# Keyteer/Mixed-precision_LU_Factorization

Measured on AMD Instinct MI355X. Metric: LU GFLOP/s at N=32768 (1/2/4/8 GPUs); IR iterations to ||r||/||b||<1e-12, higher is better.
Workload: dtype f64

## Files before the change

### mixed-precision_lu_factorization_amd/csrc/mpf_host.cpp

```cpp
#include "mpf_internal.h"
#include "../../include/MPF.h"
#include <climits>
#include <cstdio>
#include <cstdlib>
#include <cstring>
#include <cmath>
#include <iostream>
#include <vector>
#include <mutex>
#include <functional>
#include <chrono>

static thread_local std::string g_noctx_err;

namespace {
struct OptDesc { const char *name, *env; size_t off; bool wide; long long lo, hi; };
#define OPT_I(field, env, lo, hi) {#field, env, offsetof(MpfTuning, field), false, lo, hi}
#define OPT_L(field, env, lo, hi) {#field, env, offsetof(MpfTuning, field), true, lo, hi}
const OptDesc kOpts[] = {
    OPT_I(safe_pivots, "MPF_SAFE_PIVOTS", 0, 1),
    OPT_I(chain_pipeline, "MPF_CHAIN_PIPELINE", 0, 1),
    OPT_L(chain_pipeline_below, "MPF_CHAIN_PIPELINE_BELOW", 0, 1ll << 40),
    OPT_I(fp16_work32, "MPF_FP16_WORK32", 0, 1),
    OPT_I(superpanel_fp16, "MPF_SUPERPANEL", 0, 8),
    OPT_I(superpanel_fp64, "MPF_SUPERPANEL_FP64", 1, 8),
    OPT_I(no_lookahead, "MPF_NO_LOOKAHEAD", 0, 1),
    OPT_I(verbose, "MPF_VERBOSE", 0, 1),
    OPT_I(timeline, "MPF_TIMELINE", 0, 1),
    OPT_L(hp_spin_limit, "MPF_HP_SPIN_LIMIT", 1, 1ll << 31),
    OPT_L(hp_gate_ticks, "MPF_HP_GATE_TICKS", 0, 1ll << 40),
    OPT_I(hp_acq_fence, "MPF_HP_ACQ_FENCE", 0, 1),
    OPT_I(hp_window, "MPF_HP_WINDOW", -1, 1 << 30),
    OPT_I(hgemm_pad, "MPF_HGEMM_PAD", 0, 65536),
    OPT_I(hgemm_split_pad, "MPF_HGEMM_SPLIT_PAD", 0, 65536),
    OPT_I(hgemm_big, "MPF_HGEMM_BIG", 0, 1),
    OPT_I(hgemm_big_tile, "MPF_HGEMM_BIG_TILE", 0, 5),
    OPT_I(hgemm_mfma16, "MPF_HGEMM_MFMA16", 0, 1),
    OPT_I(dgemm_dma, "MPF_DGEMM_DMA", 0, 1),
    OPT_I(lazy_gather, "MPF_LAZY_GATHER", 0, 1),
    OPT_I(dpanel_fused_form, "MPF_DPANEL_FUSED", 0, 1),
    OPT_I(dist_instalments, "MPF_DIST_INSTALMENTS", 0, 1),
    OPT_L(dist_instalment_min_bytes, "MPF_DIST_INSTALMENT_MIN_BYTES", 0, 1ll << 40),
    OPT_I(generic_fused, "MPF_GENERIC_FUSED", 0, 1),
    OPT_I(fp64_rowmajor, "MPF_FP64_ROWMAJOR", 0, 1),
    OPT_L(fp64_rowmajor_min_n, "MPF_FP64_ROWMAJOR_MIN_N", 0, 1ll << 40),
    OPT_I(trsm_laswp_fused, "MPF_TRSM_LASWP_FUSED", 0, 1),
    OPT_I(fp64_two_lanes, "MPF_FP64_TWO_LANES", 0, 1 << 30),
    OPT_I(fp64_lane_a_pct, "MPF_FP64_LANE_A_PCT", 20, 90),
    OPT_I(event_timers, "MPF_EVENT_TIMERS", 0, 2),
    OPT_I(dist_world1_loop, "MPF_DIST_WORLD1_LOOP", 0, 1),
    OPT_I(gesv_fp64_tflops, "MPF_GESV_FP64_TFLOPS", 0, 1000),
    OPT_I(gate_wait_value, "MPF_GATE_WAIT_VALUE", 0, 1),
    OPT_I(host_sink, "MPF_HOST_SINK", 0, 1),
    OPT_I(sink_trace, "MPF_SINK_TRACE", 0, 1),
    OPT_I(hp_half_slabs, "MPF_HP_HALF_SLABS", 0, 1),
    OPT_I(hp_half_slabs_rows, "MPF_HP_HALF_SLABS_ROWS", 256, 32768),
    OPT_I(hp_local_xcd, "MPF_HP_LOCAL_XCD", 0, 2),
    OPT_I(host_late_parts, "MPF_HOST_LATE_PARTS", 0, 4),
    OPT_L(host_late_min_n, "MPF_HOST_LATE_MIN_N", 0, 1ll << 40),
    OPT_I(host_first_pct, "MPF_HOST_FIRST_PCT", 5, 100),
    OPT_I(host_late_q_pct, "MPF_HOST_LATE_Q_PCT", 1, 1000),
    OPT_L(host_sink_min_n, "MPF_HOST_SINK_MIN_N", 0, 1ll << 40),
    OPT_I(dist_solve_p2p, "MPF_DIST_SOLVE_P2P", 0, 1),
#ifdef MPF_PROBE
    OPT_I(hp_stamp, "MPF_HP_STAMP", 0, 1),
    OPT_I(hp_r256_upto, "MPF_HP_R256_UPTO", 0, 1 << 30),
    OPT_I(dgemm_w8, "MPF_DGEMM_W8", 0, 1),
    OPT_I(gemm_lds_pad, "MPF_GEMM_LDS_PAD", 0, 65536),
    OPT_I(hgemm_big_reg, "MPF_HGEMM_BIG_REG", 0, 1),
    OPT_I(hgemm_dbg, "MPF_HGEMM_DBG", 0, 8191),
#endif
};
#undef OPT_I
#undef OPT_L
void opt_store(MpfTuning &t, const OptDesc &d, long long v) {
    if (v < d.lo) v = d.lo;
    if (v > d.hi) v = d.hi;
    char *p = (char *)&t + d.off;
    if (d.wide) *(long long *)p = v; else *(int *)p = (int)v;
}
long long opt_load(const MpfTuning &t, const OptDesc &d) {
    const char *p = (const char *)&t + d.off;
    return d.wide ? *(const long long *)p : (long long)*(const int *)p;
}
void tuning_from_env(MpfTuning &t) {
    for (const OptDesc &d : kOpts)
        if (const char *e = getenv(d.env)) if (*e) opt_store(t, d, atoll(e));
}
}

static int fail(mpf_ctx *c, int code, const std::string &msg) {
    if (c) c->err = msg; else g_noctx_err = msg;
    return code;
}

extern "C" {

int mpf_create(mpf_ctx **out, int device) {
    if (!out) return -1;
    *out = nullptr;
    int ndev = 0;
    hipError_t e = hipGetDeviceCount(&ndev);
    if (e != hipSuccess || ndev == 0) return fail(nullptr, -3, "No HIP devices available.");
    if (device < 0 || device >= ndev) return fail(nullptr, -1, "mpf_create: bad device index");
    mpf_ctx *c = new mpf_ctx();
    tuning_from_env(c->tune);
    c->device = device;
    if (hipSetDevice(device) != hipSuccess) { delete c; return fail(nullptr, -2, "hipSetDevice failed"); }
    hipDeviceProp_t prop;
    if (hipGetDeviceProperties(&prop, device) == hipSuccess) c->num_cus = prop.multiProcessorCount;
    if (hipStreamCreateWithFlags(&c->stream, hipStreamNonBlocking) != hipSuccess) { delete c; return fail(nullptr, -2, "hipStreamCreate failed"); }
    c->own_stream = true;
    {
        int lo = 0, hi = 0;
        hipDeviceGetStreamPriorityRange(&lo, &hi);
        if (hipStreamCreateWithPriority(&c->pstream, hipStreamNonBlocking, hi) != hipSuccess) c->pstream = nullptr;
        if (hipStreamCreateWithPriority(&c->tstream, hipStreamNonBlocking, hi) != hipSuccess) c->tstream = nullptr;
    }
    if (hipMalloc((void **)&c->ws, sizeof(MpfWorkspace)) != hipSuccess) { hipStreamDestroy(c->stream); delete c; return fail(nullptr, -2, "hipMalloc(workspace) failed"); }
    hipMemset(c->ws, 0, sizeof(MpfWorkspace));
    if (hipExtMallocWithFlags((void **)&c->hp_signal, 8, hipMallocSignalMemory) != hipSuccess) { c->hp_signal = nullptr; (void)hipGetLastError(); }
    else hipMemset(c->hp_signal, 0, 8);
    hipEventCreate(&c->ev0);
    hipEventCreate(&c->ev1);
    *out = c;
    return 0;
}

int mpf_destroy(mpf_ctx *c) {
    if (!c) return 0;
    hipSetDevice(c->device);
// ... 381 lines not shown
                if (!e) e = launch_laswp_from_list(c, d_A, lda, first, c->lists);
                if (!e) e = launch_dgetf2_npv(c, d_A, lda, pr, pc, o.fused_panel, 0);
                return e;
            });
            st.panels++;
        }
    }
    for (int64_t k = 0; k < N && rc == 0; k += nb) {
        const int pc = (int)((N - k) < nb ? (N - k) : nb);
        if (N - k <= 1 || k + pc >= N) break;
        const int64_t n = N - k - pc;
        const int64_t nx = k + pc;
        const int pc2 = (int)((N - nx) < nb ? (N - nx) : nb);
        const bool has_next = (N - nx) > 1;
        double *Ap = d_A + k * lda + k;
        double *A12 = d_A + nx * lda + k;
        const int64_t ns = has_next ? pc2 : n;
        rc = ev.timed(st.ms_trsm, S, [&] { return launch_dtrsm_llnu(c, pc, ns, Ap, lda, A12, lda); });
        if (rc) break;
        rc = ev.timed(st.ms_gemm, S, [&] {
            int e = o.trailing != MPF_TRAIL_FP64 ? launch_cvt_l21(c, Ap + pc, lda, n, pc, o.trailing == MPF_TRAIL_FP16X3) : 0;
            if (!e) e = trail_gemm(c, o, n, ns, pc, Ap + pc, A12, A12 + pc, lda);
            return e; });
        if (rc) break;
        count_gemm(st, o, n, ns, pc);
        if (!has_next) break;
        hipEvent_t e1 = ev.get(), e2 = ev.get();
        hipEventRecord(e1, S);
        hipEvent_t e2p = nullptr, e2t = nullptr;
        int rcp = 0;
        const bool piped = chain_pipelined(c, ev, st, o, d_A, lda, N, nx, pc2, d_ipiv, c->lists + (nx / nb), e1, &e2p, &e2t, &rcp) == 0;
        if (piped) rc = rcp;
        else {
            hipStreamWaitEvent(P, e1, 0);
            StreamSwap sw(c, P);
            double *Anx = d_A + nx * lda + nx;
            MovedList *ml = c->lists + (nx / nb);
            rc = ev.timed(st.ms_hpanel, P, [&] {
                return launch_hgetf2(c, Anx, lda, nullptr, 0, (int)(N - nx), pc2, (int)nx, d_ipiv + nx, nullptr, 0, ml, 0, o.trailing == MPF_TRAIL_FP64 ? HP_FP64_WINDOW_ROWS : 0); });
            if (!rc) rc = ev.timed(st.ms_dpanel, P, [&] {
                int e = launch_laswp_from_list(c, d_A + nx * lda, lda, pc2, ml);
                if (!e) e = launch_dgetf2_npv(c, Anx, lda, (int)(N - nx), pc2, o.fused_panel, (int)nx);
                return e;
            });
        }
        if (rc) break;
        if (!piped) hipEventRecord(e2, P);
        st.panels++;
        if (n > pc2) {
            rc = ev.timed(st.ms_laswp, S, [&] {
                return launch_laswp_from_list(c, d_A + (nx + pc2) * lda, lda, N - nx - pc2, c->lists + (k / nb)); });
            if (rc) break;
            double *A12r = A12 + (int64_t)pc2 * lda;
            rc = ev.timed(st.ms_trsm, S, [&] { return launch_dtrsm_llnu(c, pc, n - pc2, Ap, lda, A12r, lda); });
            if (rc) break;
            if (sink) sink_notify(c, (int)(k / nb) + 1, S);
            rc = ev.timed(st.ms_gemm, S, [&] { return trail_gemm(c, o, n, n - pc2, pc, Ap + pc, A12r, A12r + pc, lda); });
            if (rc) break;
            count_gemm(st, o, n, n - pc2, pc);
        }
        if (piped) { hipStreamWaitEvent(S, e2p, 0); hipStreamWaitEvent(S, e2t, 0); }
        else hipStreamWaitEvent(S, e2, 0);
        rc = ev.timed(st.ms_laswp, S, [&] {
            const int64_t s0 = nx + pc2;
            const int64_t sw = (N - s0) < nb ? (N - s0) : nb;
            return sw > 0 ? launch_laswp_from_list(c, d_A + s0 * lda, lda, sw, c->lists + (nx / nb)) : 0;
        });
        if (o.verbose) printf("panel k=%lld rows=%lld cols=%d (look-ahead)\n", (long long)nx, (long long)(N - nx), pc2);
    }
    if (sink) {
        hipEvent_t ep = ev.get(); hipEventRecord(ep, P); hipStreamWaitEvent(S, ep, 0);
        sink_notify(c, (int)((N + nb - 1) / nb), S);
    } else if (!rc) rc = ev.timed(st.ms_laswp, S, [&] { return launch_lazy_left_swaps(c, d_A, lda, N, nb, (int)((N + nb - 1) / nb), c->lists); });
    hipError_t se = sink_stream_wait(c, S);
    hipError_t sp = sink_stream_wait(c, P);
    if (c->tstream) { const hipError_t stt = sink_stream_wait(c, c->tstream); if (sp == hipSuccess) sp = stt; }
    if (!rc && (se != hipSuccess || sp != hipSuccess))
        return fail(c, -2, std::string("factorization failed: ") + hipGetErrorString(se != hipSuccess ? se : sp));
    ev.collect();
    st.lookahead = 1;
    return rc;
}

static int factor_lookahead_rm(mpf_ctx *c, double *d_A, int64_t lda, int64_t N, int32_t nb, int32_t *d_ipiv,
                               const mpf_opts &o, mpf_stats &st) {
    hipStream_t S = c->stream, P = c->pstream, T = c->tstream;
    EvPool ev(c);
    ev.keep = &st.ms_gemm;
    int rc = 0;
    const bool sink = sink_take(c, d_A, lda, N, nb);
    double *R = c->r64;
    const int64_t ldr = N;
    LatePlan *lp = (c->late && !c->late->taken && c->late->nseg > 0 && lda == N) ? c->late : nullptr;
    if (lp) lp->taken = true;
    int lseg = 0;
    int64_t ce = lp ? lp->c0[0] : N;
    { hipEvent_t e = ev.get(); hipEventRecord(e, S); hipStreamWaitEvent(P, e, 0); if (T) hipStreamWaitEvent(T, e, 0); }
    const int pc0 = (int)(N < nb ? N : nb);
    hipEvent_t chain_a = nullptr, chain_b = nullptr;
    if (N > 1) {
        hipEvent_t e0 = ev.get();
        {
            StreamSwap sw(c, P);
            rc = ev.timed(st.ms_hpanel, P, [&] {
                int e = launch_hgetf2(c, d_A, lda, nullptr, 0, (int)N, pc0, 0, d_ipiv, nullptr, 0, c->lists, 0, o.trailing == MPF_TRAIL_FP64 ? HP_FP64_WINDOW_ROWS : 0);
                if (!e) e = launch_laswp_from_list(c, d_A, lda, pc0, c->lists);
                if (!e) e = launch_dgetf2_npv(c, d_A, lda, (int)N, pc0, o.fused_panel, 0);
                return e; });
            hipEventRecord(e0, P);
        }
        st.panels++;
        if (!rc && pc0 < ce) rc = ev.timed(st.ms_cvt, S, [&] { return launch_transpose64(c, d_A + (int64_t)pc0 * lda, lda, R + pc0, ldr, N, ce - pc0, true); });
        hipStreamWaitEvent(S, e0, 0);
        chain_a = e0;
    }
    int64_t cm = -1;
    hipEvent_t doneL = nullptr, doneR = nullptr, prevR = nullptr;
    hipEvent_t init_done = ev.get();
    hipEventRecord(init_done, S);
    bool was_two = false;
    for (int64_t k = 0; k < N && rc == 0; k += nb) {
        const int pc = (int)((N - k) < nb ? (N - k) : nb);
        if (N - k <= 1 || k + pc >= N) break;
        const int64_t n = N - k - pc;
        const int64_t nx = k + pc;
        const int pc2 = (int)((N - nx) < nb ? (N - nx) : nb);
        const bool has_next = (N - nx) > 1;
        double *Ap = d_A + k * lda + k;
        double *LT = c->rm_lt + ((k / nb) & 1) * N * (int64_t)nb;
        const int64_t ns = has_next ? pc2 : n;
        MovedList *lk = c->lists + (k / nb);
        while (lp && lseg < lp->nseg && (k / nb >= lp->q[lseg] || nx + pc2 > ce || !has_next)) {
            const int64_t c_lo = lp->c0[lseg], c_hi = lseg + 1 < lp->nseg ? lp->c0[lseg + 1] : N, w = c_hi - c_lo;
            double *LT3 = c->rm_lt + 2 * N * (int64_t)nb;
            rc = launch_late_wait(c, lp->flags + lseg, lp->seq);
            if (!rc && lp->snapshot) {
                MPF_HIP_TRY(c, hipMemcpyAsync(lp->snapshot + c_lo * N, d_A + c_lo * lda, (size_t)w * N * sizeof(double), hipMemcpyDeviceToDevice, S));
                lp->snapped[lseg] = true;
            }
            if (!rc) rc = ev.timed(st.ms_cvt, S, [&] { return launch_transpose64(c, d_A + c_lo * lda, lda, R + c_lo, ldr, N, w, true); });
            for (int64_t kj = 0; kj < k && rc == 0; kj += nb) {
                const int64_t nxj = kj + nb, nj = N - nxj;
                double *Apj = d_A + kj * lda + kj;
                const MovedList *lj = c->lists + (kj / nb);
                rc = ev.timed(st.ms_cvt, S, [&] { return launch_transpose64(c, Apj + nb, lda, LT3, nb, nj, nb, true); });
                if (!rc) rc = ev.timed(st.ms_laswp, S, [&] { return launch_laswp_from_list_rm64(c, R + c_lo, ldr, w, lj, (int64_t)LASWP_MAXMOVED * c_lo); });
                if (!rc) rc = ev.timed(st.ms_trsm, S, [&] { return launch_dtrsm_llnu_strided(c, nb, w, Apj, lda, R + kj * ldr + c_lo, ldr, 1); });
                if (!rc) rc = ev.timed(st.ms_cvt, S, [&] { return launch_transpose64(c, d_A + c_lo * lda + kj, lda, R + kj * ldr + c_lo, ldr, nb, w, false); });
                if (!rc) rc = ev.timed(st.ms_gemm, S, [&] { return launch_dgemm_minus(c, w, nj, nb, R + kj * ldr + c_lo, ldr, LT3, nb, R + nxj * ldr + c_lo, ldr); });
                count_gemm(st, o, nj, w, nb);
                if (sink && !rc && c_hi == N) sink_notify(c, (int)(kj / nb) + 1, S);
            }
            ++lseg;
            ce = lseg < lp->nseg ? lp->c0[lseg] : N;
            cm = -1;
            doneR = ev.get();
            hipEventRecord(doneR, S);
            doneL = nullptr;
        }
        if (rc) break;
        const int64_t cw = ce - nx - pc2;
        const bool pivots_fit = c->num_cus <= 0 || (N - nx + HP_R - 1) / HP_R <= (int64_t)c->num_cus * 4 / 5;
        const bool want_two = T && c->tune.fp64_two_lanes > 0 && has_next && pivots_fit && (N - nx) > c->tune.chain_pipeline_below &&
                              cw >= c->tune.fp64_two_lanes;
        bool resplit = false;
        if (!want_two) cm = -1;
        else if (cm < 0 || (cm - (nx + pc2)) * 100 < cw * (c->tune.fp64_lane_a_pct - 10)) {
            cm = nx + pc2 + ((cw * c->tune.fp64_lane_a_pct / 100 + 127) / 128) * 128;
            if (cm > ce - 128) cm = ce - 128;
            resplit = true;
        }
        if (cm >= 0) {
            const int64_t aw = cm - (nx + pc2);
            if (!was_two && k > 0) {
                doneL = ev.get();
                hipEventRecord(doneL, S);
            }
            hipEvent_t lt_ready = ev.get();
            {
                if (prevR) hipStreamWaitEvent(P, prevR, 0);
                StreamSwap sw(c, P);
                rc = ev.timed(st.ms_cvt, P, [&] { return launch_transpose64(c, Ap + pc, lda, LT, pc, n, pc, true); });
                hipEventRecord(lt_ready, P);
            }
            if (rc) break;
            hipEvent_t e1 = ev.get(), e2 = ev.get(), evA = ev.get(), evB = ev.get();
            {
                if (chain_a) hipStreamWaitEvent(T, chain_a, 0);
                if (chain_b) hipStreamWaitEvent(T, chain_b, 0);
                if (doneL) hipStreamWaitEvent(T, doneL, 0); else hipStreamWaitEvent(T, init_done, 0);
                if (resplit && doneR) hipStreamWaitEvent(T, doneR, 0);
                StreamSwap sw(c, T);
                rc = ev.timed(st.ms_laswp, T, [&] { return launch_laswp_from_list_rm64(c, R + nx, ldr, cm - nx, lk); });
                if (!rc) rc = ev.timed(st.ms_trsm, T, [&] { return launch_dtrsm_llnu_strided(c, pc, ns, Ap, lda, R + k * ldr + nx, ldr, 1); });
                hipStreamWaitEvent(T, lt_ready, 0);
                if (!rc) rc = ev.timed(st.ms_gemm, T, [&] { return launch_dgemm_minus(c, ns, n, pc, R + k * ldr + nx, ldr, LT, pc, R + nx * ldr + nx, ldr); });
                count_gemm(st, o, n, ns, pc);
                if (!rc) rc = ev.timed(st.ms_cvt, T, [&] { return launch_transpose64(c, d_A + nx * lda + nx, lda, R + nx * ldr + nx, ldr, N - nx, pc2, false); });
                hipEventRecord(e1, T);
            }
            if (rc) break;
            {
                hipStreamWaitEvent(P, e1, 0);
                if (doneR) hipStreamWaitEvent(P, doneR, 0);
// ... 323 lines not shown
            if (!rc && overlap) { e1 = ev.get(); hipEventRecord(e1, Ci); }
            if (!rc) rc = inner_step(k, pc, nx + sw_, e1c - nx - sw_, false);
            if (!rc && N - nx > 1) rc = side_chain(nx, e1, e2);
            if (!rc) rc = far_tasks_upto(it + 1);
            if (rc) break;
            if (nx >= c1 && far.on) {
                const int64_t c2 = (c1 + sbw) < N ? (c1 + sbw) : N;
                const int64_t e2c = inner_end(c2);
                if (!rc && !f64) rc = ev.timed(st.ms_cvt, S, [&] { return launch_cvt_l21(c, d_A + c0 * lda + c1, lda, N - c1, (int)(c1 - c0), split, far.img); });
                if (!rc) rc = big_update(far, e1c, e2c - e1c);
                if (!rc) rc = back_to_f64(c1, e1c, e2c - e1c);
                if (lanes) { ni_ready = ev.get(); hipEventRecord(ni_ready, S); }
                if (!rc) rc = big_update(far, e2c, N - e2c);
                if (rc) break;
            }
            if (overlap) { if (e2) { if (lanes) chain_done = e2; else hipStreamWaitEvent(S, e2, 0); } }
            if (o.verbose) printf("panel k=%lld rows=%lld (super-panel [%lld, %lld))\n", (long long)nx, (long long)(N - nx), (long long)c0, (long long)c1);
        }
        if (stop) break;
    }
    if (lanes) { hipEvent_t e = ev.get(); hipEventRecord(e, Ci); hipStreamWaitEvent(S, e, 0); if (chain_done) hipStreamWaitEvent(S, chain_done, 0); }
    if (!rc) rc = ev.timed(st.ms_laswp, S, [&] { return launch_lazy_left_swaps(c, d_A, lda, N, nb, (int)((N + nb - 1) / nb), c->lists, sb); });
    hipError_t se = hipStreamSynchronize(S);
    hipError_t sp = overlap ? hipStreamSynchronize(P) : hipSuccess;
    if (overlap && c->tstream) { const hipError_t stt = hipStreamSynchronize(c->tstream); if (sp == hipSuccess) sp = stt; }
    if (lanes) { const hipError_t sc = hipStreamSynchronize(Ci); if (sp == hipSuccess) sp = sc; }
    if (!rc && (se != hipSuccess || sp != hipSuccess))
        return fail(c, -2, std::string("factorization failed: ") + hipGetErrorString(se != hipSuccess ? se : sp));
    ev.collect();
    st.lookahead = overlap ? 1 : 0;
    return rc;
}

int mpf_ensure_rowmajor_copy(mpf_ctx *c, int64_t N, int64_t cols, int32_t nb) {
    const bool bad = c->r64.grow(N * cols) || c->rm_tmp.grow((int64_t)LASWP_MAXMOVED * cols) ||
                     c->rm_lt.grow(3 * N * (int64_t)nb);
    if (bad) {
        (void)hipGetLastError();
        c->r64.release(); c->rm_tmp.release(); c->rm_lt.release();
        return 1;
    }
    return 0;
}

int mpf_factor_setup(mpf_ctx *c, int64_t N, int32_t nb, int32_t npanels, bool lists) {
    if (lists) {
        MPF_HIP_TRY(c, c->lists.grow(npanels));
        MPF_HIP_TRY(c, c->perm_tmp.grow(N * (int64_t)(nb > HP_MAXCOLS ? nb : HP_MAXCOLS)));
        MPF_HIP_TRY(c, c->Fmap.grow(2 * N));
        MPF_HIP_TRY(c, hipMemsetAsync(c->lists, 0, (size_t)npanels * sizeof(MovedList), c->stream));
    }
    const int imax = INT_MAX;
    MPF_HIP_TRY(c, hipMemcpyAsync(&c->ws->info, &imax, sizeof(int), hipMemcpyHostToDevice, c->stream));
    MPF_HIP_TRY(c, hipMemsetAsync(&c->ws->hp_timeouts, 0, sizeof(int), c->stream));
    return 0;
}

int mpf_factor_dev(mpf_ctx *c, double *d_A, int64_t lda, int64_t N, int32_t nb, int32_t *d_ipiv, const mpf_opts *opts) {
    if (!c || !d_A || !d_ipiv) return -1;
    if (N <= 0 || nb <= 0) return fail(c, -1, "mpf_factor: N and panel width must be positive");
    if (lda < N) return fail(c, -1, "mpf_factor: lda < N");
    if (N > INT_MAX / 2) return fail(c, -1, "mpf_factor: N too large");
    if (nb > 65535) return fail(c, -1, "mpf_factor: panel width > 65535");
    mpf_opts o{};
    if (opts) o = *opts;
    if (o.trailing < MPF_TRAIL_FP64 || o.trailing > MPF_TRAIL_FP16X3) return fail(c, -1, "mpf_factor: unknown trailing mode");
    MPF_HIP_TRY(c, hipSetDevice(c->device));
    const bool force_generic = o.pivot_path == 1 || safe_pivots(c);
    const bool generic = force_generic || !hgetf2_lds_eligible(c, (int)N, (int)(nb < N ? nb : N));
    int want_sb = o.trailing != MPF_TRAIL_FP64 ? c->tune.superpanel_fp16 : c->tune.superpanel_fp64;
    if (o.trailing != MPF_TRAIL_FP64 && want_sb == 0) want_sb = (o.trailing == MPF_TRAIL_FP16 && N >= 24576) ? 6 : 4;
    if (o.superpanel > 0) want_sb = o.superpanel > 8 ? 8 : o.superpanel;
    const int sb = (!generic && !o.sync_timing && (int64_t)want_sb * nb < N) ? want_sb : 1;
    if (o.trailing != MPF_TRAIL_FP64) {
        const int64_t kimg = (int64_t)sb * nb < 8 * HP_MAXCOLS ? (int64_t)sb * nb : 8 * HP_MAXCOLS;
        int e = mpf_ensure_h_images(c, N + HP_MAXCOLS + 64, (int)kimg, sb > 1); if (e) return e;
    }
    { const int e = mpf_factor_setup(c, N, nb, (int)((N + nb - 1) / nb), !generic); if (e) return e; }
    mpf_stats st{};
    st.n = N; st.nb = nb; st.superpanel = sb;
    const bool lookahead = !o.sync_timing && !o.no_lookahead && !c->tune.no_lookahead && c->pstream != nullptr;
    const bool use_rm = !generic && sb <= 1 && lookahead && o.trailing == MPF_TRAIL_FP64 && c->tune.fp64_rowmajor &&
                        N >= c->tune.fp64_rowmajor_min_n && N > nb && mpf_ensure_rowmajor_copy(c, N, N, nb) == 0;
    if (c->late && !use_rm) {
        const int e = feed_finish(c);
        c->late = nullptr;
        if (e) return e;
    }
    MPF_HIP_TRY(c, hipEventRecord(c->ev0, c->stream));
    int rc;
    if (generic) rc = factor_generic(c, d_A, lda, N, nb, d_ipiv, o, st, force_generic);
    else if (sb > 1) rc = factor_superpanel(c, d_A, lda, N, nb, d_ipiv, o, st, sb, lookahead);
    else if (use_rm) rc = factor_lookahead_rm(c, d_A, lda, N, nb, d_ipiv, o, st);
    else if (lookahead) rc = factor_lookahead(c, d_A, lda, N, nb, d_ipiv, o, st);
    else {
        mpf_opts o2 = o;
        rc = factor_sync_timed(c, d_A, lda, N, nb, d_ipiv, o2, st);
    }
    hipEventRecord(c->ev1, c->stream);
    hipError_t se = sink_stream_wait(c, c->stream);
    if (rc) return rc;
    if (se != hipSuccess) return fail(c, -2, std::string("factorization failed: ") + hipGetErrorString(se));
    float ms = 0;
    hipEventElapsedTime(&ms, c->ev0, c->ev1);
    st.ms_total = ms;
    if (o.trailing == MPF_TRAIL_FP64 && N >= 8192 && ms > 0)
        c->fp64_rate_tflops = 2.0 / 3.0 * (double)N * (double)N * (double)N / (ms * 1e-3) / 1e12;
    int info = 0, flags0 = 0;
    MPF_HIP_TRY(c, hipMemcpy(&info, &c->ws->info, sizeof(int), hipMemcpyDeviceToHost));
    MPF_HIP_TRY(c, hipMemcpy(&flags0, &c->ws->hp_timeouts, sizeof(int), hipMemcpyDeviceToHost));
    st.info = info == INT_MAX ? 0 : info;
    st.hpanel_timeouts = flags0;
    const double h2d = c->stats.ms_h2d, d2h = c->stats.ms_d2h;
    c->stats = st;
    c->stats.ms_h2d = h2d; c->stats.ms_d2h = d2h;
    if (flags0) return fail(c, -4, "fp16 pivot kernel: inter-workgroup hand-off timed out (its workgroups were not all resident: GPU "
                                   "shared with another process?).  d_A and ipiv are invalid.  Use mpf_opts.pivot_path = 1 or MPF_SAFE_PIVOTS=1");
    return st.info;
}

static int ensure_host_copies(mpf_ctx *c, int64_t N) {
    MPF_HIP_TRY(c, c->host_A.grow(N * N));
    MPF_HIP_TRY(c, c->host_P.grow(N));
    return 0;
}

int mpf_trim(mpf_ctx *c) {
    if (!c) return -1;
    MPF_HIP_TRY(c, hipSetDevice(c->device));
    MPF_HIP_TRY(c, hipStreamSynchronize(c->stream));
    c->host_A.release(); c->host_P.release(); c->host_A0.release();
    sink_trim(c);
    feed_trim(c);
    c->r64.release(); c->rm_tmp.release(); c->rm_lt.release();
    c->w32.release();
    return 0;
}

int mpf_factor_host(mpf_ctx *c, double *A_host, int64_t N, int32_t nb, int32_t *ipiv_host, const mpf_opts *opts) {
    if (!c || !A_host || !ipiv_host) return -1;
    if (N <= 0 || nb <= 0) return fail(c, -1, "mpf_factor: N and panel width must be positive");
    MPF_HIP_TRY(c, hipSetDevice(c->device));
    { const int e = ensure_host_copies(c, N); if (e) return e; }
    double *dA = c->host_A;
    int32_t *dP = c->host_P;
    const size_t bytes = (size_t)N * (size_t)N * sizeof(double), pbytes = (size_t)N * sizeof(int32_t);
    const bool want_sink = c->tune.host_sink && N >= c->tune.host_sink_min_n && c->pstream != nullptr && !(opts && (opts->sync_timing || opts->no_lookahead)) &&
                           !(opts && opts->trailing != MPF_TRAIL_FP64) && !(opts && opts->pivot_path == 1);
    bool armed = false;
    if (want_sink) {
        if (c->host_A0.grow((int64_t)((bytes + pbytes + sizeof(double) - 1) / sizeof(double))) != hipSuccess)
            (void)hipGetLastError();
        if (c->host_A0) {
            const int e = sink_attach(c, A_host, N, nb);
            if (e < 0) return e;
            armed = e == 0;
        }
    }
    LatePlan plan;
    const int64_t npan = (N + nb - 1) / nb;
    int parts = c->tune.host_late_parts;
    if (!want_sink || !c->tune.fp64_rowmajor || N < c->tune.fp64_rowmajor_min_n || N < c->tune.host_late_min_n || npan < 32 || c->tune.no_lookahead || safe_pivots(c) ||
        !hgetf2_lds_eligible(c, (int)N, (int)nb) || c->tune.superpanel_fp64 > 1 || (opts && opts->superpanel > 1)) parts = 0;
    if (parts > 0 && !c->late_flags) {
        if (c->late_flags.grow(16) != hipSuccess) { (void)hipGetLastError(); parts = 0; }
        else memset(c->late_flags, 0, 16 * sizeof(unsigned));
    }
    if (parts > 0 && mpf_ensure_rowmajor_copy(c, N, N, nb) != 0) parts = 0;
    if (parts > 0) {
        const int64_t first = ((N * c->tune.host_first_pct / 100 + nb - 1) / nb) * nb;
        plan.nseg = parts;
        for (int i = 0; i < parts; ++i) {
            int64_t c0 = first + ((N - first) * i / parts / nb) * nb;
            if (c0 < 4 * (int64_t)nb) c0 = 4 * (int64_t)nb;
            plan.c0[i] = c0;
            plan.q[i] = 1;
            if (i && plan.c0[i] <= plan.c0[i - 1]) { plan.nseg = 0; break; }
        }
        if (plan.nseg && plan.c0[0] >= N) plan.nseg = 0;
        plan.flags = c->late_flags;
        plan.seq = ++c->late_seq;
        plan.snapshot = armed ? c->host_A0 : nullptr;
    }
    const int64_t up_cols = plan.nseg ? plan.c0[0] : N;
    const size_t up_bytes = (size_t)up_cols * (size_t)N * sizeof(double);
    hipEvent_t e0, e1;
    hipEventCreate(&e0); hipEventCreate(&e1);
    hipMemsetAsync(&c->ws->flags[1], 0, sizeof(int), c->stream);
    hipEventRecord(e0, c->stream);
    const auto t_up0 = std::chrono::steady_clock::now();
    hipMemcpyAsync(dA, A_host, up_bytes, hipMemcpyHostToDevice, c->stream);
    const double up_ms = std::chrono::duration<double, std::milli>(std::chrono::steady_clock::now() - t_up0).count();
    hipMemcpyAsync(dP, ipiv_host, pbytes, hipMemcpyHostToDevice, c->stream);
    hipEventRecord(e1, c->stream);
    if (plan.nseg) {
        double gbps = up_ms > 0 ? (double)up_bytes / up_ms / 1e6 : 45.0;
        if (gbps > 45.0) gbps = 45.0;
        if (gbps < 5.0) gbps = 5.0;
        const double fl_per_ms = 58e9, chain_ms = nb * 2.4e-3;
        double t = 0, arrive = 0;
        int64_t k = 0, ce = plan.c0[0];
        for (int i = 0; i < plan.nseg; ++i) {
            const int64_t hi = i + 1 < plan.nseg ? plan.c0[i + 1] : N, w = hi - plan.c0[i];
            arrive += (double)w * N * 8 / gbps / 1e6 * (c->tune.host_late_q_pct / 100.0);
            while (t < arrive && (k / nb + 3) * (int64_t)nb <= ce) {
                const double rows = (double)(N - k - nb), cols = (double)(ce - k - nb);
                const double upd = 2.0 * rows * cols * nb / fl_per_ms;
                t += upd > chain_ms ? upd : chain_ms;
                k += nb;
            }
            plan.q[i] = (int)(k / nb) > 0 ? (int)(k / nb) : 1;
            for (int64_t kj = 0; kj < k; kj += nb) t += 2.0 * (double)(N - kj - nb) * (double)w * nb / fl_per_ms;
            if (t < arrive) t = arrive;
            ce = hi;
        }
        if (c->tune.sink_trace) {
            fprintf(stderr, "late plan: first part %lld columns up in %.1f ms (%.1f GB/s)", (long long)plan.c0[0], up_ms, up_ms > 0 ? (double)up_bytes / up_ms / 1e6 : 0.0);
// ... 179 lines not shown
```

### mixed-precision_lu_factorization_amd/csrc/mpf_internal.h

```cpp
#pragma once
#include <hip/hip_runtime.h>
#include <stdint.h>
#include <string>
#include <vector>
#include <functional>
#include "../../include/mpf_c.h"

constexpr int HP_R = 256;
constexpr int HP_T = 512;
constexpr int HP_MAXG = 256;
constexpr int HP_MAXCOLS = 256;
constexpr int LASWP_MAXMOVED = 2 * HP_MAXCOLS;

struct MovedList {
    int n;
    int pad[3];
    int src[LASWP_MAXMOVED];
    int dst[LASWP_MAXMOVED];
};

struct MpfWorkspace {
    unsigned long long cand[2][HP_MAXG];
    int flags[16];
    unsigned long long rowbuf[2][HP_MAXG][HP_MAXCOLS / 2];
    int hp_timeouts;
    int pad0[3];
    MovedList list0;
    int info;
    int pad[3];
    unsigned long long hp_stamps[8];
    unsigned long long hp_progress;
    unsigned long long hp_xcd_target;
    unsigned long long hp_xcd_roles;
};

struct MpfTuning {
    int safe_pivots = 0;
    int chain_pipeline = 1;
    long long chain_pipeline_below = 10240;
    int fp16_work32 = 1;
    int superpanel_fp16 = 0;
    int superpanel_fp64 = 1;
    int no_lookahead = 0;
    int verbose = 0;
    int timeline = 0;
    long long hp_spin_limit = 1ll << 21;
    long long hp_gate_ticks = 200000000ll;
    int hp_window = -1;
    int hp_acq_fence = 0;
    int hgemm_pad = 0;
    int hgemm_split_pad = 32768;
    int hgemm_big = 1;
    int hgemm_mfma16 = 1;
    int hgemm_big_tile = 0;
    int dgemm_dma = 1;
    int lazy_gather = 1;
    int dpanel_fused_form = 1;
    int dist_instalments = 1;
    long long dist_instalment_min_bytes = 8ll << 20;
    int generic_fused = 1;
    int fp64_rowmajor = 1;
    long long fp64_rowmajor_min_n = 8192;
    int trsm_laswp_fused = 1;
    int fp64_two_lanes = 8192;
    int dist_solve_p2p = 0;
    int host_sink = 1;
    int hp_local_xcd = 1;
    int hp_half_slabs = 1;
    int hp_half_slabs_rows = 16384;
    int sink_trace = 0;
    int host_late_parts = 3;
    long long host_late_min_n = 16384;
    int host_first_pct = 25;
    int host_late_q_pct = 110;
    long long host_sink_min_n = 4096;
    int gate_wait_value = 0;
    int gesv_fp64_tflops = 0;
    int dist_world1_loop = 0;
    int event_timers = 1;
    int fp64_lane_a_pct = 50;
#ifdef MPF_PROBE
    int hp_stamp = 0;
    int hp_r256_upto = 1 << 30;
    int dgemm_w8 = 1;
    int gemm_lds_pad = 0;
    int hgemm_dbg = 0;
    int hgemm_big_reg = 0;
#endif
};

template <class T, bool Pinned = false>
struct Buf {
    Buf() = default;
    Buf(const Buf &) = delete;
    Buf &operator=(const Buf &) = delete;
    ~Buf() { release(); }
    hipError_t grow(int64_t n) {
        if (n <= cap_) return hipSuccess;
        release();
        void *q = nullptr;
        const hipError_t e = Pinned ? hipHostMalloc(&q, (size_t)n * sizeof(T)) : hipMalloc(&q, (size_t)n * sizeof(T));
        if (e != hipSuccess) return e;
        p_ = (T *)q;
        cap_ = n;
        return hipSuccess;
    }
    void release() {
        if (p_) (void)(Pinned ? hipHostFree(p_) : hipFree(p_));
        p_ = nullptr;
        cap_ = 0;
    }
    T *get() const { return p_; }
    operator T *() const { return p_; }
    int64_t cap() const { return cap_; }
private:
    T *p_ = nullptr;
    int64_t cap_ = 0;
};

struct mpf_ctx {
    MpfTuning tune;
    unsigned attr_done = 0;
    unsigned attr_big = 0;
    int device = 0;
    hipStream_t stream = nullptr;
    bool own_stream = false;
    hipStream_t pstream = nullptr;
    hipStream_t tstream = nullptr;
    hipStream_t xstream = nullptr;
    std::vector<hipEvent_t> ev_pool;
    MpfWorkspace *ws = nullptr;
    hipEvent_t ev0 = nullptr, ev1 = nullptr;
    std::string err;
    mpf_stats stats{};
    int num_cus = 0;
    Buf<double> solve_buf;
    int64_t solve_n = 0;
    Buf<unsigned short> h_L, h_U;
    int64_t h_rows = 0;
    Buf<unsigned short> h_Lb[2];
    int h_kmax = 0;
    unsigned hp_seq = 0;
    unsigned long long *hp_signal = nullptr;
    Buf<int32_t> perm_buf;
    Buf<MovedList> lists;
    Buf<int> Fmap;
    Buf<double> perm_tmp;
    Buf<double> trsv_inv;
    Buf<double> trsv_inv256;
    Buf<int> trsv_cnt;
    Buf<double> krylov;
    Buf<double> res_part;
    Buf<double> ext_part, ext_red, ext_vec;
    Buf<double> blk_tiles, blk_part;
    Buf<int> blk_mask;
    Buf<double> dtiles;
    Buf<float> w32;
    Buf<double> r64;
    bool hgemm_standalone = false;
    mpf_p2p_fn p2p_fn = nullptr;
    void *p2p_user = nullptr;
    double gmres_budget_ms = 0;
    double fp64_rate_tflops = 0;
    Buf<double> host_A;
    Buf<int32_t> host_P;
    Buf<double> host_A0;
    Buf<unsigned, true> late_flags;
    unsigned late_seq = 0;
    struct ColFeed *feed = nullptr;
    struct LatePlan *late = nullptr;
    struct RowSink *sink = nullptr;
    Buf<double> rm_tmp;
    Buf<double> rm_lt;
    Buf<unsigned short> g16;
    Buf<unsigned long long> gcand;
    void *rccl_comm = nullptr;
    int rccl_rank = 0, rccl_world = 0;
    long long rccl_bcast_calls = 0, rccl_bcast_bytes = 0, rccl_allreduce_calls = 0, rccl_p2p_calls = 0, rccl_p2p_bytes = 0;
    Buf<double> dist_buf[2];
    Buf<float> dist_w32;
    Buf<double> dist_spl;
    int hp_resident_per_cu = -1;
    int hp_win_per_cu = 0;
    int hp_full_beside_waiter = 0;
    int hp_win_beside_waiter = 0;
};

#define MPF_HIP_TRY(ctx, expr)                                                        \
    do {                                                                              \
        hipError_t e_ = (expr);                                                       \
        if (e_ != hipSuccess) {                                                       \
            (ctx)->err = std::string(#expr) + ": " + hipGetErrorString(e_);           \
            return -2;                                                                \
        }                                                                             \
    } while (0)

enum { ATTR_HP = 1, ATTR_DGEMM = 2, ATTR_HGEMM = 4, ATTR_HGEMM256 = 8, ATTR_HGEMM_PP = 16, ATTR_HGEMM16_BIG32 = 32, ATTR_HGEMM16_BIG64 = 64 };
inline bool safe_pivots(const mpf_ctx *c) { return c->tune.safe_pivots != 0; }

int launch_double_to_fp16(mpf_ctx *c, const double *in, uint16_t *out, int64_t n);
int launch_hdiv(mpf_ctx *c, const uint16_t *a, const uint16_t *b, uint16_t *q, int64_t n);
int launch_hgetf2(mpf_ctx *c, const double *A64, int64_t lda, uint16_t *P16, int64_t ld16, int rows,
                  int cols, int ipiv_offset, int *d_ipiv, uint16_t *out16, int64_t ldo, MovedList *moved, int waiters = 0, int prefer_window_rows = 0);
bool hgetf2_lds_eligible(mpf_ctx *c, int rows, int cols);
bool hgetf2_fits_beside(mpf_ctx *c, int rows, int cols, int waiters);
long long hgetf2_capacity_rows(mpf_ctx *c, int waiters, int form = 0);
int laswp_gated_footprint(int *lds_bytes, int *vgprs, int *threads);
int laswp_gated_grid(int64_t ncols);
constexpr int HP_FP64_WINDOW_ROWS = 20000;
int hp_query_residency(mpf_ctx *c);
int launch_hgetf2_gate(mpf_ctx *c, int target);
int launch_laswp_block(mpf_ctx *c, double *A, int64_t lda, int64_t ncols, int k, int cols, const int *d_ipiv, int64_t nrows);
int launch_laswp_block_gated(mpf_ctx *c, double *A, int64_t lda, int64_t ncols, int k, int cols, const int *d_ipiv, int64_t nrows, int target);
int dgetf2_npv_pieces(mpf_ctx *c, int cols);
int launch_dgetf2_npv_piece(mpf_ctx *c, double *P, int64_t ld, int rows, int cols, int fused, int info_base, int piece);
int launch_dpanel_tile_copy(mpf_ctx *c, double *dst, int64_t ld, int piece);
int launch_hgetf2_generic(mpf_ctx *c, const double *A64, int64_t lda, uint16_t *P16, int64_t ld16, int rows, int cols,
                          int ipiv_offset, int *d_ipiv, uint16_t *out16, int64_t ldo);
int launch_laswp_seq(mpf_ctx *c, double *A, int64_t lda, int64_t ncols, int k, int cols, const int *d_ipiv, int64_t nrows);
int launch_laswp_from_list(mpf_ctx *c, double *A, int64_t lda, int64_t ncols, const MovedList *ml);
int launch_laswp_from_list_hole(mpf_ctx *c, double *A, int64_t lda, int64_t ncols, const MovedList *ml, int64_t hole_from, int64_t hole_len);
int launch_lazy_left_swaps(mpf_ctx *c, double *A, int64_t lda, int64_t N, int nb, int npanels, const MovedList *lists, int sb = 1,
                           int world = 1, int rank = 0);
struct LatePlan {
    int nseg = 0;
    int64_t c0[4] = {0, 0, 0, 0};
    int q[4] = {0, 0, 0, 0};
    unsigned *flags = nullptr;
    unsigned seq = 0;
    double *snapshot = nullptr;
    bool taken = false;
    bool snapped[4] = {false, false, false, false};
};
int launch_late_wait(mpf_ctx *c, const unsigned *flag, unsigned seq);
int feed_start(mpf_ctx *c, const double *A_host, double *d_A, int64_t N, LatePlan *lp);
int feed_finish(mpf_ctx *c);
void feed_destroy(mpf_ctx *c);
void feed_trim(mpf_ctx *c);
int sink_attach(mpf_ctx *c, double *A_host, int64_t N, int nb);
bool sink_take(mpf_ctx *c, const double *d_A, int64_t lda, int64_t N, int nb);
void sink_notify(mpf_ctx *c, int upto_panel, hipStream_t stream);
hipError_t sink_stream_wait(mpf_ctx *c, hipStream_t stream);
int sink_finish(mpf_ctx *c, int *panels_sent);
void sink_destroy(mpf_ctx *c);
void sink_trim(mpf_ctx *c);
int launch_laswp(mpf_ctx *c, double *A, int64_t lda, int64_t ncols, int k, int cols, const int *d_ipiv);
int launch_laswp_plan(mpf_ctx *c, const int *d_ipiv, int k, int cols, MovedList *out);
int launch_dgetf2_npv(mpf_ctx *c, double *P, int64_t ld, int rows, int cols, int fused, int info_base);
int launch_dtrsm_llnu(mpf_ctx *c, int m, int64_t n, const double *L, int64_t ldl, double *B, int64_t ldb);
int launch_dgemm_minus(mpf_ctx *c, int64_t m, int64_t n, int k, const double *A, int64_t lda,
                       const double *B, int64_t ldb, double *C, int64_t ldc);
int launch_cvt_l21(mpf_ctx *c, const double *A, int64_t lda, int64_t m, int K, int split, int img = 0, int64_t elem_off = 0);
int launch_hgemm_minus(mpf_ctx *c, int64_t m, int64_t n, int K, const double *B, int64_t ldb, double *C, int64_t ldc,
                       int split, int img = 0, int64_t elem_off = 0);
int launch_hgemm_minus_w32(mpf_ctx *c, int64_t m, int64_t n, int K, const double *B, int64_t ldb, float *C, int64_t ldc,
                           int split, int img = 0, int64_t elem_off = 0);
// ... 114 lines not shown
```

Before: 53430.

## Pair consecutive FP64 panels so the far trailing update runs with K=2nb

```diff
diff --git a/mixed-precision_lu_factorization_amd/csrc/mpf_host.cpp b/mixed-precision_lu_factorization_amd/csrc/mpf_host.cpp
--- a/mixed-precision_lu_factorization_amd/csrc/mpf_host.cpp
+++ b/mixed-precision_lu_factorization_amd/csrc/mpf_host.cpp
@@ -47,6 +47,8 @@
     OPT_I(trsm_laswp_fused, "MPF_TRSM_LASWP_FUSED", 0, 1),
     OPT_I(fp64_two_lanes, "MPF_FP64_TWO_LANES", 0, 1 << 30),
     OPT_I(fp64_lane_a_pct, "MPF_FP64_LANE_A_PCT", 20, 90),
+    OPT_I(fp64_pair, "MPF_FP64_PAIR", 0, 1),
+    OPT_L(fp64_pair_min_n, "MPF_FP64_PAIR_MIN_N", 0, 1ll << 40),
     OPT_I(event_timers, "MPF_EVENT_TIMERS", 0, 2),
     OPT_I(dist_world1_loop, "MPF_DIST_WORLD1_LOOP", 0, 1),
     OPT_I(gesv_fp64_tflops, "MPF_GESV_FP64_TFLOPS", 0, 1000),
@@ -594,8 +596,185 @@
     return rc;
 }
 
+struct PairHandover {
+    int64_t k0 = 0;
+    hipEvent_t chain = nullptr;
+    hipEvent_t doneL = nullptr, doneR = nullptr;
+    int64_t cm = -1;
+};
+
+static int factor_rm_pairs(mpf_ctx *c, EvPool &ev, mpf_stats &st, const mpf_opts &o, double *d_A, int64_t lda, int64_t N, int32_t nb,
+                           int32_t *d_ipiv, hipEvent_t init_done, PairHandover &h) {
+    hipStream_t S = c->stream, P = c->pstream, T = c->tstream;
+    double *R = c->r64;
+    const int64_t ldr = N, ldp = 2 * (int64_t)nb;
+    const int pref_win = HP_FP64_WINDOW_ROWS;
+    int rc = 0;
+    hipEvent_t doneX = nullptr, doneA = nullptr, doneB = nullptr;
+    int64_t cm = -1;
+    int64_t k = h.k0;
+    struct { bool valid = false; int64_t k = 0, c_lo = 0, w = 0; double *PI2 = nullptr; hipEvent_t ready = nullptr; } pendB;
+    auto far_update = [&](int64_t kk, double *pi2, int64_t c_lo, int64_t w) -> int {
+        const int64_t r0 = kk + 2 * (int64_t)nb;
+        const int e = ev.timed(st.ms_gemm, S, [&] { return launch_dgemm_minus(c, w, N - r0, 2 * nb, R + kk * ldr + c_lo, ldr, pi2, ldp, R + r0 * ldr + c_lo, ldr); });
+        count_gemm(st, o, N - r0, w, 2 * nb);
+        return e;
+    };
+    auto flush_B = [&](hipEvent_t ps) -> int {
+        if (!pendB.valid) return 0;
+        hipStreamWaitEvent(S, pendB.ready, 0);
+        if (ps) hipStreamWaitEvent(S, ps, 0);
+        const int e = far_update(pendB.k, pendB.PI2, pendB.c_lo, pendB.w);
+        doneB = ev.get();
+        hipEventRecord(doneB, S);
+        pendB.valid = false;
+        return e;
+    };
+    for (; rc == 0; k += 2 * (int64_t)nb) {
+        const int64_t k1 = k + nb, k2 = k1 + nb, k3 = k2 + nb, k5 = k3 + 2 * (int64_t)nb;
+        if (k5 + 256 > N || (N - k1) <= c->tune.fp64_pair_min_n) break;
+        if (c->num_cus > 0 && (N - k1 + HP_R - 1) / HP_R > (int64_t)c->num_cus * 4 / 5) break;
+        const int64_t cw = N - k5;
+        bool resplit = false;
+        if (cm < 0 || (cm - k5) * 100 < cw * (c->tune.fp64_lane_a_pct - 10)) {
+            cm = k5 + ((cw * c->tune.fp64_lane_a_pct / 100 + 127) / 128) * 128;
+            if (cm > N - 128) cm = N - 128;
+            resplit = true;
+        }
+        double *Ak = d_A + k * lda + k, *Ak1 = d_A + k1 * lda + k1;
+        double *PI = c->rm_pair + ((k / (2 * nb)) & 1) * N * ldp;
+        double *PI2 = PI + (int64_t)nb * ldp;
+        const MovedList *lk = c->lists + (k / nb), *lk1 = c->lists + (k1 / nb);
+        hipEvent_t lt_ready = ev.get(), e1 = ev.get(), inner_done = ev.get(), chain1 = ev.get(), pi_ready = ev.get(), e2 = ev.get(),
+                   chain2 = ev.get(), evX = ev.get(), evA = ev.get(), evB = ev.get(), ps1 = ev.get(), ps2 = ev.get();
+        {
+            if (doneB) hipStreamWaitEvent(P, doneB, 0);
+            StreamSwap sw(c, P);
+            rc = ev.timed(st.ms_cvt, P, [&] { return launch_transpose64(c, Ak + nb, lda, PI, ldp, N - k1, nb, true); });
+            hipEventRecord(lt_ready, P);
+        }
+        if (rc) break;
+        {
+            hipStreamWaitEvent(T, h.chain, 0);
+            hipStreamWaitEvent(T, doneX ? doneX : init_done, 0);
+            StreamSwap sw(c, T);
+            rc = ev.timed(st.ms_laswp, T, [&] { return launch_laswp_from_list_rm64(c, R + k1, ldr, k3 - k1, lk, (int64_t)LASWP_MAXMOVED * k1); });
+            if (!rc) rc = ev.timed(st.ms_trsm, T, [&] { return launch_dtrsm_llnu_strided(c, nb, nb, Ak, lda, R + k * ldr + k1, ldr, 1); });
+            hipStreamWaitEvent(T, lt_ready, 0);
+            if (!rc) rc = ev.timed(st.ms_gemm, T, [&] { return launch_dgemm_minus(c, nb, N - k1, nb, R + k * ldr + k1, ldr, PI, ldp, R + k1 * ldr + k1, ldr); });
+            count_gemm(st, o, N - k1, nb, nb);
+            if (!rc) rc = ev.timed(st.ms_cvt, T, [&] { return launch_transpose64(c, Ak1, lda, R + k1 * ldr + k1, ldr, N - k1, nb, false); });
+            hipEventRecord(e1, T);
+            if (!rc) rc = ev.timed(st.ms_trsm, T, [&] { return launch_dtrsm_llnu_strided(c, nb, nb, Ak, lda, R + k * ldr + k2, ldr, 1); });
+            if (!rc) rc = ev.timed(st.ms_gemm, T, [&] { return launch_dgemm_minus(c, nb, N - k1, nb, R + k * ldr + k2, ldr, PI, ldp, R + k1 * ldr + k2, ldr); });
+            count_gemm(st, o, N - k1, nb, nb);
+            if (!rc) rc = ev.timed(st.ms_cvt, T, [&] { return launch_transpose64(c, d_A + k1 * lda + k, lda, R + k * ldr + k1, ldr, nb, k3 - k1, false); });
+            hipEventRecord(inner_done, T);
+        }
+        if (rc) break;
+        {
+            hipStreamWaitEvent(P, e1, 0);
+            if (doneA) hipStreamWaitEvent(P, doneA, 0);
+            hipEventRecord(ps1, P);
+            StreamSwap sw(c, P);
+            rc = ev.timed(st.ms_hpanel, P, [&] {
+                return launch_hgetf2(c, Ak1, lda, nullptr, 0, (int)(N - k1), nb, (int)k1, d_ipiv + k1, nullptr, 0, c->lists + (k1 / nb), 0, pref_win); });
+            if (!rc) rc = ev.timed(st.ms_dpanel, P, [&] {
+                int e = launch_laswp_from_list(c, d_A + k1 * lda, lda, nb, lk1);
+                if (!e) e = launch_dgetf2_npv(c, Ak1, lda, (int)(N - k1), nb, o.fused_panel, (int)k1);
+                return e; });
+            hipEventRecord(chain1, P);
+            st.panels++;
+            hipStreamWaitEvent(P, inner_done, 0);
+            if (!rc) rc = ev.timed(st.ms_laswp, P, [&] { return launch_laswp_from_list_rm64(c, PI - k1 * ldp, ldp, nb, lk1, 0); });
+            if (!rc) rc = ev.timed(st.ms_cvt, P, [&] { return launch_transpose64(c, Ak1 + nb, lda, PI2 + nb, ldp, N - k2, nb, true); });
+            hipEventRecord(pi_ready, P);
+        }
+        if (!rc) rc = flush_B(ps1);
+        if (rc) break;
+        {
+            hipStreamWaitEvent(T, chain1, 0);
+            StreamSwap sw(c, T);
+            rc = ev.timed(st.ms_laswp, T, [&] { return launch_laswp_from_list_rm64(c, R + k2, ldr, nb, lk1, (int64_t)LASWP_MAXMOVED * k2); });
+            if (!rc) rc = ev.timed(st.ms_trsm, T, [&] { return launch_dtrsm_llnu_strided(c, nb, nb, Ak1, lda, R + k1 * ldr + k2, ldr, 1); });
+            hipStreamWaitEvent(T, pi_ready, 0);
+            if (!rc) rc = ev.timed(st.ms_gemm, T, [&] { return launch_dgemm_minus(c, nb, N - k2, nb, R + k1 * ldr + k2, ldr, PI2 + nb, ldp, R + k2 * ldr + k2, ldr); });
+            count_gemm(st, o, N - k2, nb, nb);
+            if (!rc) rc = ev.timed(st.ms_cvt, T, [&] { return launch_transpose64(c, d_A + k2 * lda + k2, lda, R + k2 * ldr + k2, ldr, N - k2, nb, false); });
+            hipEventRecord(e2, T);
+            if (!rc) rc = ev.timed(st.ms_cvt, T, [&] { return launch_transpose64(c, d_A + k2 * lda + k1, lda, R + k1 * ldr + k2, ldr, nb, nb, false); });
+        }
+        if (rc) break;
+        {
+            hipStreamWaitEvent(P, e2, 0);
+            if (doneB) hipStreamWaitEvent(P, doneB, 0);
+            hipEventRecord(ps2, P);
+            StreamSwap sw(c, P);
+            double *Ak2 = d_A + k2 * lda + k2;
+            MovedList *ml = c->lists + (k2 / nb);
+            rc = ev.timed(st.ms_hpanel, P, [&] {
+                return launch_hgetf2(c, Ak2, lda, nullptr, 0, (int)(N - k2), nb, (int)k2, d_ipiv + k2, nullptr, 0, ml, 0, pref_win); });
+            if (!rc) rc = ev.timed(st.ms_dpanel, P, [&] {
+                int e = launch_laswp_from_list(c, d_A + k2 * lda, lda, nb, ml);
+                if (!e) e = launch_dgetf2_npv(c, Ak2, lda, (int)(N - k2), nb, o.fused_panel, (int)k2);
+                return e; });
+            hipEventRecord(chain2, P);
+            st.panels++;
+        }
+        if (rc) break;
+        auto far_prep = [&](int64_t c_lo, int64_t w) -> int {
+            const int64_t off = (int64_t)LASWP_MAXMOVED * c_lo;
+            int e = ev.timed(st.ms_laswp, T, [&] {
+                int e2_ = launch_laswp_from_list_rm64(c, R + c_lo, ldr, w, lk, off);
+                if (!e2_) e2_ = launch_laswp_from_list_rm64(c, R + c_lo, ldr, w, lk1, off);
+                return e2_; });
+            if (!e) e = ev.timed(st.ms_trsm, T, [&] { return launch_dtrsm_llnu_strided(c, nb, w, Ak, lda, R + k * ldr + c_lo, ldr, 1); });
+            if (!e) e = ev.timed(st.ms_gemm, T, [&] { return launch_dgemm_minus(c, w, nb, nb, R + k * ldr + c_lo, ldr, PI, ldp, R + k1 * ldr + c_lo, ldr); });
+            count_gemm(st, o, nb, w, nb);
+            if (!e) e = ev.timed(st.ms_trsm, T, [&] { return launch_dtrsm_llnu_strided(c, nb, w, Ak1, lda, R + k1 * ldr + c_lo, ldr, 1); });
+            if (!e) e = ev.timed(st.ms_cvt, T, [&] { return launch_transpose64(c, d_A + c_lo * lda + k, lda, R + k * ldr + c_lo, ldr, 2 * nb, w, false); });
+            return e;
+        };
+        {
+            if (doneA) hipStreamWaitEvent(T, doneA, 0); else hipStreamWaitEvent(T, init_done, 0);
+            if (resplit && doneB) hipStreamWaitEvent(T, doneB, 0);
+            StreamSwap sw(c, T);
+            rc = far_prep(k3, k5 - k3);
+            hipEventRecord(evX, T);
+            if (!rc) rc = far_prep(k5, cm - k5);
+            hipEventRecord(evA, T);
+        }
+        if (rc) break;
+        hipStreamWaitEvent(S, evX, 0);
+        hipStreamWaitEvent(S, ps2, 0);
+        rc = far_update(k, PI2, k3, k5 - k3);
+        if (rc) break;
+        doneX = ev.get();
+        hipEventRecord(doneX, S);
+        hipStreamWaitEvent(S, evA, 0);
+        rc = far_update(k, PI2, k5, cm - k5);
+        if (rc) break;
+        doneA = ev.get();
+        hipEventRecord(doneA, S);
+        {
+            if (doneB) hipStreamWaitEvent(T, doneB, 0);
+            StreamSwap sw(c, T);
+            rc = far_prep(cm, N - cm);
+            hipEventRecord(evB, T);
+        }
+        if (rc) break;
+        pendB.valid = true; pendB.k = k; pendB.PI2 = PI2; pendB.c_lo = cm; pendB.w = N - cm; pendB.ready = evB;
+        h.chain = chain2;
+        if (o.verbose) printf("panels k=%lld, %lld rows=%lld (row-major copy, paired: far update K = %d, lanes split at %lld)\n", (long long)k1, (long long)k2, (long long)(N - k1), 2 * nb, (long long)cm);
+    }
+    if (!rc) rc = flush_B(nullptr);
+    h.k0 = k;
+    h.doneL = doneA; h.doneR = doneB; h.cm = cm;
+    return rc;
+}
+
 static int factor_lookahead_rm(mpf_ctx *c, double *d_A, int64_t lda, int64_t N, int32_t nb, int32_t *d_ipiv,
-                               const mpf_opts &o, mpf_stats &st) {
+                               const mpf_opts &o, mpf_stats &st, bool pairs) {
     hipStream_t S = c->stream, P = c->pstream, T = c->tstream;
     EvPool ev(c);
     ev.keep = &st.ms_gemm;
@@ -631,7 +810,17 @@
     hipEvent_t init_done = ev.get();
     hipEventRecord(init_done, S);
     bool was_two = false;
-    for (int64_t k = 0; k < N && rc == 0; k += nb) {
+    int64_t k0 = 0;
+    if (pairs && !rc && !sink && !lp && T && N > 1) {
+        PairHandover h;
+        h.chain = chain_a;
+        rc = factor_rm_pairs(c, ev, st, o, d_A, lda, N, nb, d_ipiv, init_done, h);
+        if (h.k0 > 0) {
+            k0 = h.k0; chain_a = h.chain; doneL = h.doneL; doneR = h.doneR; cm = h.cm;
+            was_two = true;
+        }
+    }
+    for (int64_t k = k0; k < N && rc == 0; k += nb) {
         const int pc = (int)((N - k) < nb ? (N - k) : nb);
         if (N - k <= 1 || k + pc >= N) break;
         const int64_t n = N - k - pc;
@@ -1121,6 +1310,9 @@
     const bool lookahead = !o.sync_timing && !o.no_lookahead && !c->tune.no_lookahead && c->pstream != nullptr;
     const bool use_rm = !generic && sb <= 1 && lookahead && o.trailing == MPF_TRAIL_FP64 && c->tune.fp64_rowmajor &&
                         N >= c->tune.fp64_rowmajor_min_n && N > nb && mpf_ensure_rowmajor_copy(c, N, N, nb) == 0;
+    bool use_pairs = use_rm && c->tune.fp64_pair && c->tune.fp64_two_lanes > 0 && c->tstream && nb % 16 == 0 && N > c->tune.fp64_pair_min_n;
+    if (use_pairs && c->num_cus > 0 && (N - nb + HP_R - 1) / HP_R > (int64_t)c->num_cus * 4 / 5) use_pairs = false;
+    if (use_pairs && c->rm_pair.grow(4 * N * (int64_t)nb) != hipSuccess) { (void)hipGetLastError(); use_pairs = false; }
     if (c->late && !use_rm) {
         const int e = feed_finish(c);
         c->late = nullptr;
@@ -1130,7 +1322,7 @@
     int rc;
     if (generic) rc = factor_generic(c, d_A, lda, N, nb, d_ipiv, o, st, force_generic);
     else if (sb > 1) rc = factor_superpanel(c, d_A, lda, N, nb, d_ipiv, o, st, sb, lookahead);
-    else if (use_rm) rc = factor_lookahead_rm(c, d_A, lda, N, nb, d_ipiv, o, st);
+    else if (use_rm) rc = factor_lookahead_rm(c, d_A, lda, N, nb, d_ipiv, o, st, use_pairs);
     else if (lookahead) rc = factor_lookahead(c, d_A, lda, N, nb, d_ipiv, o, st);
     else {
         mpf_opts o2 = o;
@@ -1171,7 +1363,7 @@
     c->host_A.release(); c->host_P.release(); c->host_A0.release();
     sink_trim(c);
     feed_trim(c);
-    c->r64.release(); c->rm_tmp.release(); c->rm_lt.release();
+    c->r64.release(); c->rm_tmp.release(); c->rm_lt.release(); c->rm_pair.release();
     c->w32.release();
     return 0;
 }
diff --git a/mixed-precision_lu_factorization_amd/csrc/mpf_internal.h b/mixed-precision_lu_factorization_amd/csrc/mpf_internal.h
--- a/mixed-precision_lu_factorization_amd/csrc/mpf_internal.h
+++ b/mixed-precision_lu_factorization_amd/csrc/mpf_internal.h
@@ -79,6 +79,8 @@
     int dist_world1_loop = 0;
     int event_timers = 1;
     int fp64_lane_a_pct = 50;
+    int fp64_pair = 1;
+    long long fp64_pair_min_n = 16384;
 #ifdef MPF_PROBE
     int hp_stamp = 0;
     int hp_r256_upto = 1 << 30;
@@ -172,6 +174,7 @@
     struct RowSink *sink = nullptr;
     Buf<double> rm_tmp;
     Buf<double> rm_lt;
+    Buf<double> rm_pair;
     Buf<unsigned short> g16;
     Buf<unsigned long long> gcand;
     void *rccl_comm = nullptr;
```

After: 54660, median of 6. 1.02x the previous value.
